# janelia-flyem/flypylib

Hardware: AMD Instinct MI355X
Metric: inference Mvoxels/sec, vgg_like (rf 18, 22^3 coarse -> 88^3 per reference tile), synthetic EM uint8 volume (higher is better)
Workload: dtype f16s; 1 GPU; the 520^3 volume of BASELINE.json's metric (configs[0]'s substack size) per GPU: vgg_like inference, 520x520x520 synthetic uint8 volume, reference tile lattice 102^3 (pitch 88), u8 in / f32 out resident in HBM; tile_in=102, executor=vgg_split_f16, parallelism=z-slab tile sharding x1, no collective, device=AMD Radeon Graphics (gfx950:sramecc+:xnack-)

## Files before the change

flypylib_amd/csrc/vgg_split.hip:

```cpp
#define FPL_F16 1
#include <algorithm>
#include <cmath>

#include "fast_paths.h"
#include "mfma_util.h"
#include "pack_weights.h"
#include <type_traits>
#include "vgg_split_lds.h"
#include "vgg_tiles.h"

namespace {

constexpr int CH = 48;
constexpr int CHP = 24, NPASS = CH / CHP;
constexpr int LO_OFF = CHP * 2;
constexpr int PASS_BYTES = 2 * LO_OFF;
constexpr int VOX = NPASS * PASS_BYTES;
constexpr int KS = (27 * CHP + 31) / 32;
constexpr int KTAB = (KS + 4) / 4 * 4;
constexpr int KTAB_BYTES = 4 * KTAB * 4;
static_assert(CHP % 8 == 0, "a lane's 8 k-slots stay inside one tap");

__host__ __device__ constexpr int64_t chan_off(int ch, int64_t plane) { return (ch / CHP) * plane + (ch % CHP) * 2; }

__device__ __forceinline__ h16x8 pack_relu_split_x(const f32x4 &blk) {
  u32x4 v;
  Pair2 p;
  p = split_pk_relu(blk[0], blk[1]); v[0] = p.hi; v[2] = p.lo;
  p = split_pk_relu(blk[2], blk[3]); v[1] = p.hi; v[3] = p.lo;
  return __builtin_bit_cast(h16x8, v);
}
__device__ __forceinline__ h16x8 pack_relu_split_x(const f32x4 &blk, unsigned &ovf) {
  const h16x8 r = pack_relu_split_x(blk);
  const u32x4 v = __builtin_bit_cast(u32x4, r);
  ovf_note(ovf, pk_max_i16(v[0], v[1]));
  return r;
}

__device__ __forceinline__ f32x4 chain48(const h16x8 (&w)[4], const Frag2 &h01, h16x8 hx, f32x4 acc) {
  acc = mfma16(w[1], h01.hi, acc);
  acc = mfma16(w[0], h01.lo, acc);
  acc = mfma16(w[2], hx, acc);
  acc = mfma16(w[3], hx, acc);
  return mfma16(w[0], h01.hi, acc);
}

__device__ __forceinline__ void store_split12(unsigned char *vox, int64_t plane, int g, const f32x4 (&v)[3],
                                              unsigned &ovf) {
  unsigned hi[6], lo[6];
#pragma unroll
  for (int b = 0; b < 3; ++b) {
    const Pair2 p0 = split_pk(v[b][0], v[b][1], ovf), p1 = split_pk(v[b][2], v[b][3], ovf);
    hi[2 * b] = p0.hi; hi[2 * b + 1] = p1.hi;
    lo[2 * b] = p0.lo; lo[2 * b + 1] = p1.lo;
  }
  unsigned char *d = vox + (g >> 1) * plane + 24 * (g & 1);
  *reinterpret_cast<u32x4_a8 *>(d) = u32x4_a8{hi[0], hi[1], hi[2], hi[3]};
  *reinterpret_cast<u32x2 *>(d + 16) = u32x2{hi[4], hi[5]};
  *reinterpret_cast<u32x4_a8 *>(d + LO_OFF) = u32x4_a8{lo[0], lo[1], lo[2], lo[3]};
  *reinterpret_cast<u32x2 *>(d + LO_OFF + 16) = u32x2{lo[4], lo[5]};
}

constexpr int S_PZ = 4, S_PY = 8, S_PX = 32;
constexpr int S_TZ = 2 * S_PZ + 2, S_TY = 2 * S_PY + 2, S_TX = 2 * S_PX + 2;
constexpr int S_TP = 80;
constexpr int S_TILE = S_TZ * S_TY * S_TP;
constexpr int S_WAVES = 8;
constexpr int S_ROWS = S_TZ * S_TY;
constexpr int S_WROWS = (S_ROWS + S_WAVES - 1) / S_WAVES;
constexpr int S_TASKS = S_PZ * S_PY * 2 / S_WAVES;
constexpr int S_RPT = 3;
static_assert(S_RPT * S_TASKS >= S_WROWS && S_WROWS <= 64, "stem fill schedule");
constexpr int S_SHTAB = 64 * 48;
constexpr int S_SH2 = 4 * 12;
constexpr int S_SMEM = 4 * S_TILE * 2 + 256 * 4 + S_SHTAB * 4 + 2 * S_SH2 * 4;

struct StemSArgs {
  const void *src;
  int64_t SZ, SY, SX;
  int64_t z_hi;
  float mean, sd;
  float c0;
  const float *shtab;
  int64_t p1z0;
  const h16x8 *w1, *w2;
  const float *shift1, *shift2;
  x8::Tensor p1;
  int nbx, nby, nbz;
  int trim;
  unsigned *flag;
  float xlim;
// ... 507 lines not shown
constexpr int WQ = 2;

template <typename Fill, typename SubOff>
__device__ __forceinline__ void conv3s_kloop_f(Fill fill, unsigned char *tile,
                                               const unsigned *kofftab, const unsigned char *wglobal,
                                               unsigned vbase, SubOff sub_off, f32x4 (&acc)[4][3],
                                               int tid) {
  const int lane = tid & 63, wave = tid >> 6, g = lane >> 4;
  const unsigned *ktab = kofftab + g * KTAB;
#pragma unroll 1
  for (int pass = 0; pass < NPASS; ++pass) {
    if (pass) __syncthreads();
    fill(pass);
    const unsigned char *wl = wglobal + (size_t)pass * KS * 6 * 1024 + lane * 16;
    h16x8 wq[WQ][6];
#pragma unroll
    for (int d = 0; d < WQ; ++d)
#pragma unroll
      for (int f = 0; f < 6; ++f)
        wq[d][f] = *reinterpret_cast<const h16x8 *>(wl + (size_t)(d * 6 + f) * 1024);
    __syncthreads();
    u32x4 kv = *reinterpret_cast<const u32x4 *>(ktab);
    Frag2 bcur[4], bnxt[4];
#pragma unroll
    for (int sub = 0; sub < 4; ++sub) {
      const unsigned char *p = tile + vbase + kv[0] + sub_off(sub);
      bcur[sub].hi = *reinterpret_cast<const h16x8 *>(p);
      bcur[sub].lo = *reinterpret_cast<const h16x8 *>(p + LO_OFF);
    }
#pragma unroll
    for (int s = 0; s < KS; ++s) {
      if ((s + 1) % 4 == 0) kv = *reinterpret_cast<const u32x4 *>(ktab + s + 1);
      const unsigned koff = kv[(s + 1) % 4];
#pragma unroll
      for (int sub = 0; sub < 4; ++sub) {
        const unsigned char *p = tile + vbase + koff + sub_off(sub);
        bnxt[sub].hi = *reinterpret_cast<const h16x8 *>(p);
        bnxt[sub].lo = *reinterpret_cast<const h16x8 *>(p + LO_OFF);
      }
      __builtin_amdgcn_s_setprio(1);
#pragma unroll
      for (int sub = 0; sub < 4; ++sub)
#pragma unroll
        for (int b = 0; b < 3; ++b) acc[sub][b] = mfma16(wq[s % WQ][3 + b], bcur[sub].hi, acc[sub][b]);
#pragma unroll
      for (int sub = 0; sub < 4; ++sub)
#pragma unroll
        for (int b = 0; b < 3; ++b) acc[sub][b] = mfma16(wq[s % WQ][b], bcur[sub].lo, acc[sub][b]);
#pragma unroll
      for (int sub = 0; sub < 4; ++sub)
#pragma unroll
        for (int b = 0; b < 3; ++b) acc[sub][b] = mfma16(wq[s % WQ][b], bcur[sub].hi, acc[sub][b]);
      __builtin_amdgcn_s_setprio(0);
      if (s + WQ < KS) {
#pragma unroll
        for (int f = 0; f < 6; ++f)
          wq[s % WQ][f] = *reinterpret_cast<const h16x8 *>(wl + (size_t)((s + WQ) * 6 + f) * 1024);
      }
#pragma unroll
      for (int sub = 0; sub < 4; ++sub) bcur[sub] = bnxt[sub];
    }
  }
}

template <int TZ, int TY, int TX, typename SubOff>
__device__ __forceinline__ void conv3s_kloop(const unsigned char *act, int AZ, int AY, int AX,
                                             int z0, int y0, int x0, unsigned char *tile,
                                             const unsigned *kofftab, const unsigned char *wglobal,
                                             unsigned vbase, SubOff sub_off, f32x4 (&acc)[4][3],
                                             int tid) {
  const int lane = tid & 63, wave = tid >> 6;
  auto fill = [&](int pass) {
    stage_tile<TZ, TY, TX, PASS_BYTES, PASS_BYTES>(act + (int64_t)pass * AZ * AY * AX * PASS_BYTES, AZ, AY, AX,
                                                   z0, y0, x0, tile, wave, lane);
  };
  conv3s_kloop_f(fill, tile, kofftab, wglobal, vbase, sub_off, acc, tid);
}

constexpr int M_TZ = 6, M_TY = 6, M_TX = 18;
constexpr int M_TILE_BYTES = ((M_TZ * M_TY * M_TX * PASS_BYTES + 1023) / 1024) * 1024;
constexpr int M_SMEM = M_TILE_BYTES + KTAB_BYTES;
static_assert(2 * M_SMEM <= 160 * 1024, "two workgroups must fit one CU");

struct MidXArgs {
  x8::Tensor p1;
  const unsigned char *w3;
  const h16x8 *w4;
  const float *shift3, *shift4;
  x8::Tensor p2;
  x8::Walk walk;
  unsigned *flag;
};

__global__ __launch_bounds__(64 * x8::WAVES, 2) void vggs_mid_pool(MidXArgs a) {
  unsigned *ktab = reinterpret_cast<unsigned *>(smem + 2 * x8::BUF);
  const int tid = threadIdx.x, lane = tid & 63;
  const int wave = __builtin_amdgcn_readfirstlane(tid >> 6);
  const int c = lane & 15, g = lane >> 4;
  x8::ktab_init(ktab, tid);
  const x8::TileDma td = x8::tile_dma_init(wave, lane, a.p1.Y, a.p1.XP, (unsigned)a.p1.part_bytes());
  const int S = (int)gridDim.x >> 3, nbricks = a.walk.bricks();
  const int group = (int)blockIdx.x & 7, slot = (int)blockIdx.x >> 3;
  x8::Cursor cur;
  if (!x8::cursor_first(a.walk, nbricks, group, slot, S, cur)) return;
  const int64_t part = a.p1.part_bytes();
  auto origin = [&](const x8::Cursor &q) {
    return a.p1.p + a.p1.vox(8 * q.bz, 4 * q.by, 16 * q.bx) * 16;
  };
  const int pzl = wave >> 1, pyl = wave & 1;
  const unsigned vb = (unsigned)(((2 * pzl) * x8::ZS + (2 * pyl) * x8::TX + c) * 16);
  auto sub_off = [](int sub) -> unsigned { return (unsigned)((((sub >> 1) & 1) * x8::ZS + (sub & 1) * x8::TX) * 16); };
  unsigned ovf_all = 0u;
  x8::prime(smem, td, origin(cur), part, a.w3, wave, lane);
  for (;;) {
    x8::Cursor nxt = cur;
    const bool has_next = x8::cursor_next(a.walk, slot, S, nxt);
    int zero = 0;
    asm volatile("" : "+s"(zero));
    f32x4 acc[4][3];
#pragma unroll
    for (int b = 0; b < 3; ++b) {
      const f32x4 sh = *reinterpret_cast<const f32x4 *>(a.shift3 + zero + 16 * b + 4 * g);
#pragma unroll
      for (int sub = 0; sub < 4; ++sub) acc[sub][b] = sh;
    }
    x8::conv_block(smem, ktab + 8 * g, td, origin(cur), origin(has_next ? nxt : cur), part, a.w3, vb,
                   sub_off, wave, lane, acc);
    asm volatile("" : "+s"(zero));
    const h16x8 *w4p = a.w4 + zero;
    f32x4 sh4[3];
#pragma unroll
    for (int b = 0; b < 3; ++b)
#pragma unroll
      for (int r = 0; r < 4; ++r) sh4[b][r] = a.shift4[zero + x8::out_channel(b, g, r)];
    h16x8 w4[3][4];
#pragma unroll
    for (int s = 0; s < 4; ++s)
#pragma unroll
      for (int b = 0; b < 3; ++b) w4[b][s] = w4p[(s * 3 + b) * 64 + lane];
    f32x4 pooled[3] = {{0.f, 0.f, 0.f, 0.f}, {0.f, 0.f, 0.f, 0.f}, {0.f, 0.f, 0.f, 0.f}};
    unsigned ovf = 0u;
#pragma unroll
    for (int sub = 0; sub < 4; ++sub) {
      const Frag2 h0 = pack_relu_split(acc[sub][0], acc[sub][1], ovf);
      const h16x8 hx = pack_relu_split_x(acc[sub][2], ovf);
#pragma unroll
      for (int b = 0; b < 3; ++b) {
        const f32x4 a4 = chain48(w4[b], h0, hx, sh4[b]);
#pragma unroll
        for (int r = 0; r < 4; ++r) pooled[b][r] = __builtin_fmaxf(pooled[b][r], a4[r]);
      }
    }
#pragma unroll
    for (int b = 0; b < 3; ++b)
#pragma unroll
      for (int r = 0; r < 4; ++r)
        pooled[b][r] = __builtin_fmaxf(pooled[b][r], __shfl_xor(pooled[b][r], 1));
    const int pz = 4 * cur.bz + pzl, py = 2 * cur.by + pyl, px = 8 * cur.bx + (c >> 1);
    const bool inside = pz < a.p2.Z && py < a.p2.Y && px < a.p2.X;
    if ((c & 1) == 0 && inside)
      x8::store12(a.p2, a.p2.vox(pz, py, px), g, pooled, ovf);
    ovf_all = pk_max_i16(ovf_all, inside ? ovf : 0u);
    if (!has_next) break;
    cur = nxt;
  }
  ovf_commit(ovf_all, a.flag, FPL_RANGE_MID);
}

constexpr int T_W7 = 3 * 6, T_W8 = 3;
__device__ __forceinline__ void head_chain(const f32x4 (&acc)[4][3], const unsigned char *w6p,
                                           const unsigned char *w7p, const unsigned char *w8p, const float *sh6p,
                                           const float *sh7p, float bias8, int lane, unsigned &ovf, float (&logit)[4]) {
  const int c = lane & 15, g = lane >> 4;
  auto frag = [&](const unsigned char *w, int part_, int nfrag, int f) {
    return *reinterpret_cast<const h16x8 *>(w + ((size_t)(part_ * nfrag + f) * 64 + lane) * 16);
  };
#pragma unroll
  for (int sp = 0; sp < 2; ++sp) {
    Frag2 h5[2];
    h16x8 h5x[2];
#pragma unroll
    for (int q = 0; q < 2; ++q) {
      h5[q] = pack_relu_split(acc[2 * sp + q][0], acc[2 * sp + q][1], ovf);
      h5x[q] = pack_relu_split_x(acc[2 * sp + q][2], ovf);
    }
    Frag2 h6[2][3];
#pragma unroll
    for (int s = 0; s < 3; ++s) {
      f32x4 a6[2][2];
#pragma unroll
      for (int bb = 0; bb < 2; ++bb) {
        const int b = 2 * s + bb;
        f32x4 sh;
#pragma unroll
        for (int r = 0; r < 4; ++r) sh[r] = sh6p[16 * b + 4 * g + r];
        h16x8 w6[4];
#pragma unroll
        for (int t = 0; t < 4; ++t) w6[t] = frag(w6p, 0, 0, t * 6 + b);
#pragma unroll
        for (int q = 0; q < 2; ++q) a6[q][bb] = chain48(w6, h5[q], h5x[q], sh);
      }
#pragma unroll
      for (int q = 0; q < 2; ++q) h6[q][s] = pack_relu_split(a6[q][0], a6[q][1], ovf);
    }
    f32x4 a8[2] = {{0.f, 0.f, 0.f, 0.f}, {0.f, 0.f, 0.f, 0.f}};
#pragma unroll
    for (int s = 0; s < 3; ++s) {
      f32x4 a7[2][2];
#pragma unroll
      for (int bb = 0; bb < 2; ++bb) {
        const int b = 2 * s + bb;
        f32x4 sh;
#pragma unroll
        for (int r = 0; r < 4; ++r) sh[r] = sh7p[16 * b + 4 * g + r];
#pragma unroll
        for (int q = 0; q < 2; ++q) a7[q][bb] = sh;
#pragma unroll
        for (int t = 0; t < 3; ++t) {
          const h16x8 wh = frag(w7p, 0, T_W7, t * 6 + b), wl = frag(w7p, 1, T_W7, t * 6 + b);
#pragma unroll
          for (int q = 0; q < 2; ++q) a7[q][bb] = mfma3(wh, wl, h6[q][t], a7[q][bb]);
        }
      }
      const h16x8 w8h = frag(w8p, 0, T_W8, s), w8l = frag(w8p, 1, T_W8, s);
#pragma unroll
      for (int q = 0; q < 2; ++q) a8[q] = mfma3(w8h, w8l, pack_relu_split(a7[q][0], a7[q][1], ovf), a8[q]);
    }
#pragma unroll
    for (int q = 0; q < 2; ++q) logit[2 * sp + q] = __shfl(a8[q][0], c) + bias8;
    __builtin_amdgcn_sched_barrier(0);
  }
}

struct TailSArgs {
  const unsigned char *p2;
  int P2Z, P2Y, P2X;
  const unsigned char *w5;
  const float *shift5;
  int CZ, CY, CX;
  const unsigned char *w6, *w7, *w8;
  const float *shift6, *shift7;
  float bias8;
// ... 28 lines not shown
  }
  auto sub_off = [](int sub) -> unsigned { return (unsigned)(sub * M_TX * PASS_BYTES); };
  conv3s_kloop<M_TZ, M_TY, M_TX>(a.p2, a.P2Z, a.P2Y, a.P2X, cz0, cy0, cx0, tile, kofftab, a.w5,
                                 vbase, sub_off, acc, tid);

  float logit[4];
  unsigned ovf = 0u;
  head_chain(acc, a.w6, a.w7, a.w8, a.shift6, a.shift7, a.bias8, lane, ovf, logit);
  ovf_commit(ovf, a.flag, FPL_RANGE_TAIL);

  const int cz = cz0 + wave, cx = cx0 + c;
#pragma unroll
  for (int sub = 0; sub < 4; ++sub) {
    const int cy = cy0 + sub;
    const float p = 1.f / (1.f + expf(-logit[sub]));
    if (cz < a.CZ && cy < a.CY && cx < a.CX) {
      const int64_t fz0 = 4 * (a.gz0 + cz), fy = 4 * (int64_t)cy + g, fx0 = 4 * (int64_t)cx;
      if (fy < a.VY && fx0 < a.VX) {
        const int nx = (int)(a.VX - fx0 < 4 ? a.VX - fx0 : 4);
#pragma unroll
        for (int dz = 0; dz < 4; ++dz) {
          const int64_t fz = fz0 + dz;
          if (fz >= a.VZ) break;
          float *o = a.dst + ((fz + a.off) * a.DY + fy + a.off) * a.DX + fx0 + a.off;
          if (nx == 4) {
            *reinterpret_cast<f32x4_a4 *>(o) = f32x4_a4{p, p, p, p};
          } else {
            for (int i = 0; i < nx; ++i) o[i] = p;
          }
        }
      }
    }
  }
}

struct TailXArgs {
  x8::Tensor p2;
  const unsigned char *w5;
  const float *shift5;
  int CZ, CY, CX;
  const unsigned char *w6, *w7, *w8;
  const float *shift6, *shift7;
  float bias8;
  float *dst;
  int64_t DY, DX;
  int64_t gz0;
  int64_t VZ, VY, VX;
  int off;
  x8::Walk walk;
  unsigned *flag;
};

__global__ __launch_bounds__(64 * x8::WAVES, 2) void vggs_c5_tail(TailXArgs a) {
  unsigned *ktab = reinterpret_cast<unsigned *>(smem + 2 * x8::BUF);
  const int tid = threadIdx.x, lane = tid & 63;
  const int wave = __builtin_amdgcn_readfirstlane(tid >> 6);
  const int c = lane & 15, g = lane >> 4;
  x8::ktab_init(ktab, tid);
  const x8::TileDma td = x8::tile_dma_init(wave, lane, a.p2.Y, a.p2.XP, (unsigned)a.p2.part_bytes());
  const int S = (int)gridDim.x >> 3, nbricks = a.walk.bricks();
  const int group = (int)blockIdx.x & 7, slot = (int)blockIdx.x >> 3;
  x8::Cursor cur;
  if (!x8::cursor_first(a.walk, nbricks, group, slot, S, cur)) return;
  const int64_t part = a.p2.part_bytes();
  auto origin = [&](const x8::Cursor &q) {
    return a.p2.p + a.p2.vox(8 * q.bz, 4 * q.by, 16 * q.bx) * 16;
  };
  const unsigned vb = (unsigned)((wave * x8::ZS + c) * 16);
  auto sub_off = [](int sub) -> unsigned { return (unsigned)(sub * x8::TX * 16); };
  unsigned ovf_all = 0u;
  x8::prime(smem, td, origin(cur), part, a.w5, wave, lane);
  for (;;) {
    x8::Cursor nxt = cur;
    const bool has_next = x8::cursor_next(a.walk, slot, S, nxt);
    int zero = 0;
    asm volatile("" : "+s"(zero));
    f32x4 acc[4][3];
#pragma unroll
    for (int b = 0; b < 3; ++b) {
      const f32x4 sh = *reinterpret_cast<const f32x4 *>(a.shift5 + zero + 16 * b + 4 * g);
#pragma unroll
      for (int sub = 0; sub < 4; ++sub) acc[sub][b] = sh;
    }
    x8::conv_block(smem, ktab + 8 * g, td, origin(cur), origin(has_next ? nxt : cur), part, a.w5, vb,
                   sub_off, wave, lane, acc);

    unsigned ovf = 0u;
    float logit[4];
    asm volatile("" : "+s"(zero));
    head_chain(acc, a.w6 + zero, a.w7 + zero, a.w8 + zero, a.shift6 + zero, a.shift7 + zero, a.bias8, lane, ovf,
               logit);

    const int cz = 8 * cur.bz + wave, cx = 16 * cur.bx + c;
#pragma unroll
    for (int sub = 0; sub < 4; ++sub) {
      const int cy = 4 * cur.by + sub;
      const float p = 1.f / (1.f + expf(-logit[sub]));
      if (cz < a.CZ && cy < a.CY && cx < a.CX) {
        const int64_t fz0 = 4 * (a.gz0 + cz), fy = 4 * (int64_t)cy + g, fx0 = 4 * (int64_t)cx;
        if (fy < a.VY && fx0 < a.VX) {
          const int nx = (int)(a.VX - fx0 < 4 ? a.VX - fx0 : 4);
#pragma unroll
          for (int dz = 0; dz < 4; ++dz) {
            const int64_t fz = fz0 + dz;
            if (fz >= a.VZ) break;
            float *o = a.dst + ((fz + a.off) * a.DY + fy + a.off) * a.DX + fx0 + a.off;
            if (nx == 4) {
              *reinterpret_cast<f32x4_a4 *>(o) = f32x4_a4{p, p, p, p};
            } else {
              for (int i = 0; i < nx; ++i) o[i] = p;
            }
          }
        }
      }
    }
    ovf_all = pk_max_i16(ovf_all, ovf);
    if (!has_next) break;
    cur = nxt;
  }
  ovf_commit(ovf_all, a.flag, FPL_RANGE_TAIL);
}

constexpr int V2_RZ = M_TZ + 2, V2_RY = M_TY + 2, V2_RX = M_TX + 2;
constexpr int V2_NRAW = V2_RZ * V2_RY * V2_RX;
static_assert(V2_NRAW % 256 == 0, "raw tile pieces per thread");
constexpr int V2_SMEM = M_TILE_BYTES + KTAB_BYTES + V2_NRAW * 4 + 256 * 4;
static_assert(2 * V2_SMEM <= 160 * 1024, "two vgg_like2 workgroups must fit one CU");

struct V2SArgs {
  const void *src;
  int64_t SZ, SY, SX;
  float mean, sd;
  int64_t gz0;
  const h16x8 *wstem;
  const float *shstem;
  float c0;
  const float *shtab;
  const unsigned char *in;
  int IZ, IY, IX;
  const unsigned char *w;
  const float *shift;
  unsigned char *out;
  int OZ, OY, OX;
  BlockGrid bg;
  unsigned *flag;
  float xlim;
};

template <bool STEM, bool POOL, typename SRC>
__global__ __launch_bounds__(256, 2) void vggs2_conv3(V2SArgs a) {
  unsigned char *tile = smem;
  unsigned *kofftab = reinterpret_cast<unsigned *>(smem + M_TILE_BYTES);
  unsigned *rawt = reinterpret_cast<unsigned *>(smem + M_TILE_BYTES + KTAB_BYTES);
  unsigned *lut = rawt + V2_NRAW;
  const int tid = threadIdx.x, lane = tid & 63, wave = tid >> 6;
  const int c = lane & 15, g = lane >> 4;
  int xb, yb, zb;
  if (!brick_coords(a.bg, xb, yb, zb)) return;
  const int x0 = xb * 16, y0 = yb * 4, z0 = zb * 4;
  if (tid < 4 * KTAB) kofftab[tid] = kslot_entry<M_TY, M_TX>(tid);
  int toff[8];
  unsigned ovf = 0u, xmax = 0u;
  if (STEM) {
    auto norm_bits = [&](float raw) -> unsigned {
      const float x = (raw - a.mean) / a.sd;
      const unsigned ax = __builtin_bit_cast(unsigned, x) & 0x7FFFFFFFu;
      xmax = ax > xmax ? ax : xmax;
// ... 496 lines not shown
  if (fpl_vgg_variant(prog) == 2)
    return split2_infer(ctx, st, src, src_dtype, mean, sd, dims, origins, out_sz, zb, ze, dst);
  hipStream_t stream = ctx->stream;
  const int64_t SZ = dims[0], SY = dims[1], SX = dims[2];
  const int64_t VZ = SZ - 14, VY = SY - 14, VX = SX - 14;
  if (VZ <= 0 || VY <= 0 || VX <= 0 || zb >= ze) return 0;
  const int64_t fz_lo = (int64_t)origins[0][zb] - 7;
  const int64_t fz_hi = std::min<int64_t>((int64_t)origins[0][ze - 1] - 7 + out_sz[0], VZ);
  const int64_t cz_lo = fz_lo / 4, cz_hi = ceil_div64(fz_hi, 4);
  const int CY = (int)ceil_div64(VY, 4), CX = (int)ceil_div64(VX, 4);
  const int P2Y = CY + 2, P2X = CX + 2, P1Y = 2 * P2Y + 2, P1X = 2 * P2X + 2;
  const int P1XP = x8_pitch(P1X), P2XP = x8_pitch(P2X);
  const int64_t p1_row_bytes = (int64_t)P1Y * P1XP * VOX;
  const char *budget_env = getenv("FPL_VGG_SCRATCH_MB");
  const int64_t budget = budget_env ? (int64_t)atoll(budget_env) << 20 : (int64_t)64 << 30;
  int64_t cz_chunk = std::max<int64_t>(4, (budget / p1_row_bytes - 6) / 2);
  cz_chunk = std::min<int64_t>(cz_chunk, cz_hi - cz_lo);
  cz_chunk = (cz_chunk + 3) / 4 * 4;
  const char *edge_env = getenv("FPL_VGG_EDGE_BLOCKS");
  const int edge_blocks = edge_env ? atoi(edge_env) != 0 : 1;
  FPL_REQUIRE(ctx, (int64_t)S_TZ * SY * SX < ((int64_t)1 << 31),
              "vgg split path: a %lld x %lld plane is too large for the stem's 31-bit row "
              "offsets", (long long)SY, (long long)SX);
  {
    const int64_t max_rows = (((int64_t)1 << 32) / 16 / ((int64_t)P1Y * P1XP) - (x8::TZ + 2));
    FPL_REQUIRE(ctx, max_rows >= 14,
                "vgg split path: a %lld x %lld plane is too large for the tile loader's 32-bit "
                "offsets", (long long)SY, (long long)SX);
    cz_chunk = std::min<int64_t>(cz_chunk, std::max<int64_t>(4, ((max_rows - 6) / 2) / 4 * 4));
  }
  DevTemp tmp(ctx);
  unsigned *flag;
  FPL_TRY(fpl_range_flag(ctx, &flag));
  x8::Tensor p1 = {nullptr, (int)(2 * cz_chunk + 6), P1Y, P1X, P1XP}, p2 = {nullptr, (int)(cz_chunk + 2), P2Y, P2X, P2XP};
  void *p1v, *p2v;
  FPL_TRY(tmp.alloc((size_t)(p1.bytes() + p1.slack_bytes()), &p1v));
  FPL_TRY(tmp.alloc((size_t)(p2.bytes() + p2.slack_bytes()), &p2v));
  void *dumpv;
  FPL_TRY(tmp.alloc(256, &dumpv));
  const unsigned pgrid = (unsigned)std::max(8, ctx->n_cu / 8 * 8);
  const unsigned char *F = st->frags;
  const float *S = st->shifts;
  for (int64_t c0 = cz_lo; c0 < cz_hi; c0 += cz_chunk) {
    const int CZ = (int)std::min<int64_t>(cz_chunk, cz_hi - c0);
    const int P2Z = CZ + 2, P1Z = 2 * P2Z + 2;
    p1 = x8::Tensor{(unsigned char *)p1v, P1Z, P1Y, P1X, P1XP};
    p2 = x8::Tensor{(unsigned char *)p2v, P2Z, P2Y, P2X, P2XP};
    FPL_HIP(ctx, hipMemsetAsync(p1.p + p1.bytes(), 0, (size_t)p1.slack_bytes(), stream));
    FPL_HIP(ctx, hipMemsetAsync(p2.p + p2.bytes(), 0, (size_t)p2.slack_bytes(), stream));
    {
      StemSArgs a;
      a.src = src; a.SZ = SZ; a.SY = SY; a.SX = SX; a.mean = mean; a.sd = sd;
      a.p1z0 = 2 * c0;
      a.z_hi = std::min<int64_t>(SZ, 4 * (c0 + CZ) + 14);
      a.w1 = (const h16x8 *)(F + st->off_w[0]);
      a.w2 = (const h16x8 *)(F + st->off_w[1]);
      a.shift1 = S + st->off_s[0]; a.shift2 = S + st->off_s[1];
      a.c0 = 0.f; a.shtab = nullptr;
      if (src_dtype == FPL_U8) {
        a.w1 = (const h16x8 *)st->w1_int; a.shtab = st->shift1_int;
        a.c0 = st->int_c0;
      }
      a.p1 = p1;
      a.flag = flag; a.xlim = st->xlim; a.dump = (unsigned char *)dumpv;
      a.nbx = (int)ceil_div64(P1X, S_PX); a.nby = (int)ceil_div64(P1Y, S_PY);
      a.nbz = (int)ceil_div64(P1Z, S_PZ);
      a.trim = edge_blocks;
      const unsigned grid = (unsigned)std::min<int64_t>((int64_t)a.nbx * a.nby * a.nbz,
                                                        (int64_t)ctx->n_cu);
      TimedLaunch tl(ctx, "vggs_stem_pool");
      if (src_dtype == FPL_U8)
        vggs_stem_pool<uint8_t><<<grid, 64 * S_WAVES, S_SMEM, stream>>>(a);
      else
        vggs_stem_pool<float><<<grid, 64 * S_WAVES, S_SMEM, stream>>>(a);
    }
    {
      MidXArgs a;
      a.p1 = p1;
      a.w3 = F + st->off_w[2];
      a.w4 = (const h16x8 *)(F + st->off_w[3]);
      a.shift3 = S + st->off_s[2]; a.shift4 = S + st->off_s[3];
      a.p2 = p2;
      a.flag = flag;
      a.walk = x8::Walk{(int)ceil_div64(P2X, 8), (int)ceil_div64(P2Y, 2), (int)ceil_div64(P2Z, 4)};
      TimedLaunch tl(ctx, "vggs_mid_pool");
      vggs_mid_pool<<<pgrid, 64 * x8::WAVES, x8::SMEM, stream>>>(a);
    }
    {
      TailXArgs a;
      a.p2 = p2;
      a.w5 = F + st->off_w[4]; a.shift5 = S + st->off_s[4];
      a.CZ = CZ; a.CY = CY; a.CX = CX;
      a.w6 = F + st->off_w[5]; a.w7 = F + st->off_w[6]; a.w8 = F + st->off_w[7];
      a.shift6 = S + st->off_s[5]; a.shift7 = S + st->off_s[6]; a.bias8 = st->bias8;
      a.dst = dst; a.DY = SY; a.DX = SX; a.gz0 = c0;
      a.VZ = std::min<int64_t>(fz_hi, VZ); a.VY = VY; a.VX = VX; a.off = 7;
      a.flag = flag;
      a.walk = x8::Walk{(int)ceil_div64(CX, 16), (int)ceil_div64(CY, 4), (int)ceil_div64(CZ, 8)};
      TimedLaunch tl(ctx, "vggs_c5_tail");
      vggs_c5_tail<<<pgrid, 64 * x8::WAVES, x8::SMEM, stream>>>(a);
    }
    FPL_HIP(ctx, hipGetLastError());
  }
  return 0;
}
```

flypylib_amd/csrc/vgg_split_lds.h:

```cpp
#pragma once
#include "mfma_util.h"
#include "vgg_tiles.h"

namespace x8 {

constexpr int CQ = 8, NQ = 6;
constexpr int KQ = 7;
constexpr int BZ = 8, BY = 4, BX = 16;
constexpr int TZ = BZ + 2, TY = BY + 2, TX = BX + 2;
constexpr int ZS = 118;
constexpr int PLANE = (TZ - 1) * ZS + TY * TX;
constexpr int CHUNKS = (2 * PLANE + 63) / 64;
constexpr int TILE_BYTES = CHUNKS * 1024;
constexpr int WFRAGS = KQ * 6;
constexpr int WBYTES = WFRAGS * 1024;
constexpr int BUF = TILE_BYTES + WBYTES;
constexpr int KTAB_BYTES = 4 * 8 * 4;
constexpr int SMEM = 2 * BUF + KTAB_BYTES;
constexpr int WAVES = 8;
constexpr int TCH = (CHUNKS + WAVES - 1) / WAVES;
constexpr int WCH = (WFRAGS + WAVES - 1) / WAVES;
static_assert((ZS - 2 * TX - 2) % 16 == 0 && (TX - 2) % 16 == 0, "conflict-free tap offsets");
static_assert(SMEM <= 160 * 1024, "one workgroup per CU");
static_assert(PLANE % 2 == 0, "");

struct Tensor {
  unsigned char *p;
  int Z, Y, X;
  int XP;
  __host__ __device__ int64_t part_bytes() const { return (int64_t)Z * Y * XP * 16; }
  __host__ __device__ int64_t pass_bytes() const { return 2 * part_bytes(); }
  __host__ __device__ int64_t bytes() const { return NQ * pass_bytes(); }
  __host__ __device__ int64_t slack_bytes() const { return ((int64_t)(TZ + 1) * Y * XP + 64) * 16; }
  __host__ __device__ int64_t vox(int z, int y, int x) const { return ((int64_t)z * Y + y) * XP + x; }
};

struct Walk {
  int nbx, nby, nbz;
  __host__ __device__ int bricks() const { return ((nbx + 3) / 4) * ((nby + 3) / 4) * ((nbz + 1) / 2); }
};

struct TileDma {
  unsigned off[TCH];
};
__device__ __forceinline__ TileDma tile_dma_init(int wave, int lane, int SY, int SX, unsigned part_bytes) {
  TileDma d;
#pragma unroll
  for (int i = 0; i < TCH; ++i) {
    int slot = 64 * (wave + WAVES * i) + lane;
    slot = slot < 2 * PLANE ? slot : 2 * PLANE - 1;
    const int part = slot >= PLANE;
    const int s = slot - part * PLANE;
    const int tz = s / ZS;
    int rem = s - tz * ZS;
    rem = rem < TY * TX ? rem : TY * TX - 1;
    const int ty = rem / TX, tx = rem - ty * TX;
    d.off[i] = (unsigned)(((tz * SY + ty) * SX + tx) * 16) + (part ? part_bytes : 0u);
  }
  return d;
}

constexpr int NCH = CHUNKS + WFRAGS;
constexpr int DCH = (NCH + WAVES - 1) / WAVES;
constexpr int HCH = DCH / 2;
static_assert(TCH == 5 && 8 * 4 + 4 < CHUNKS && 8 * 4 + 5 >= CHUNKS, "chunk deal: i = 4 splits at wave 5");
static_assert(DCH % 2 == 0, "two batches");
__device__ __forceinline__ void dma_batch(const TileDma &d, int half, int wave, int lane, const unsigned char *org,
                                          const unsigned char *wpass, unsigned char *buf) {
#pragma unroll
  for (int k = 0; k < HCH; ++k) {
    const int i = HCH * half + k;
    int j = wave + WAVES * i;
    j = j < NCH ? j : NCH - 1;
    const bool tile = i < TCH - 1 || (i < TCH && j < CHUNKS);
    const unsigned char *base = tile ? org : wpass + (j - CHUNKS) * 1024;
    const unsigned off = tile ? d.off[i < TCH ? i : 0] : (unsigned)lane * 16u;
    glds16(base + off, buf + j * 1024);
  }
}

__device__ __forceinline__ void ktab_init(unsigned *ktab, int tid) {
  if (tid < 32) {
    const int g = tid >> 3, s = tid & 7;
    const int tap = 4 * s + g;
    ktab[tid] = tap < 27 ? (unsigned)(((tap / 9) * ZS + ((tap / 3) % 3) * TX + tap % 3) * 16) : 0u;
  }
}

template <typename SubOff, typename Issue>
__device__ __forceinline__ void pass_kloop(const unsigned char *buf, const unsigned *ktab_g, unsigned vb,
                                           SubOff sub_off, Issue issue, int lane, f32x4 (&acc)[4][3]) {
  const unsigned char *wl = buf + TILE_BYTES + lane * 16;
  const u32x4 k0 = *reinterpret_cast<const u32x4 *>(ktab_g), k1 = *reinterpret_cast<const u32x4 *>(ktab_g + 4);
  Frag2 bcur[4], bnxt[4];
  h16x8 wcur[6], wnxt[6];
#pragma unroll
  for (int sub = 0; sub < 4; ++sub) {
    const unsigned char *p = buf + vb + k0[0] + sub_off(sub);
    bcur[sub].hi = *reinterpret_cast<const h16x8 *>(p);
    bcur[sub].lo = *reinterpret_cast<const h16x8 *>(p + PLANE * 16);
  }
#pragma unroll
  for (int f = 0; f < 6; ++f) wcur[f] = *reinterpret_cast<const h16x8 *>(wl + f * 1024);
#pragma unroll
  for (int s = 0; s < KQ; ++s) {
    __builtin_amdgcn_sched_barrier(0);
    __builtin_amdgcn_s_setprio(1);
#pragma unroll
    for (int sub = 0; sub < 4; ++sub)
#pragma unroll
      for (int b = 0; b < 3; ++b) acc[sub][b] = mfma16(wcur[3 + b], bcur[sub].hi, acc[sub][b]);
    __builtin_amdgcn_sched_barrier(0);
    if (s + 1 < KQ) {
      const unsigned koff = s + 1 < 4 ? k0[(s + 1) & 3] : k1[(s + 1) & 3];
#pragma unroll
      for (int sub = 0; sub < 4; ++sub) {
        const unsigned char *p = buf + vb + koff + sub_off(sub);
        bnxt[sub].hi = *reinterpret_cast<const h16x8 *>(p);
        bnxt[sub].lo = *reinterpret_cast<const h16x8 *>(p + PLANE * 16);
      }
    }
    __builtin_amdgcn_sched_barrier(0);
#pragma unroll
    for (int sub = 0; sub < 4; ++sub)
#pragma unroll
      for (int b = 0; b < 3; ++b) acc[sub][b] = mfma16(wcur[b], bcur[sub].lo, acc[sub][b]);
    __builtin_amdgcn_sched_barrier(0);
    if (s + 1 < KQ) {
#pragma unroll
      for (int f = 0; f < 6; ++f) wnxt[f] = *reinterpret_cast<const h16x8 *>(wl + ((s + 1) * 6 + f) * 1024);
    }
    issue(s);
    __builtin_amdgcn_sched_barrier(0);
#pragma unroll
    for (int sub = 0; sub < 4; ++sub)
#pragma unroll
      for (int b = 0; b < 3; ++b) acc[sub][b] = mfma16(wcur[b], bcur[sub].hi, acc[sub][b]);
    __builtin_amdgcn_s_setprio(0);
    __builtin_amdgcn_sched_barrier(0);
    if (s + 1 < KQ) {
#pragma unroll
      for (int sub = 0; sub < 4; ++sub) bcur[sub] = bnxt[sub];
#pragma unroll
      for (int f = 0; f < 6; ++f) wcur[f] = wnxt[f];
    }
  }
}

template <typename SubOff>
__device__ __forceinline__ void conv_block(unsigned char *smem, const unsigned *ktab_g, const TileDma &td,
                                           const unsigned char *org_cur, const unsigned char *org_nxt,
                                           int64_t part_bytes, const unsigned char *wglobal, unsigned vb,
                                           SubOff sub_off, int wave, int lane, f32x4 (&acc)[4][3]) {
#pragma unroll 1
  for (int pp = 0; pp < NQ / 2; ++pp) {
#pragma unroll
    for (int h = 0; h < 2; ++h) {
      const int pass = 2 * pp + h;
      unsigned char *buf = smem + h * BUF, *other = smem + (h ^ 1) * BUF;
      const bool more = pass + 1 < NQ;
      const unsigned char *torg = more ? org_cur + (int64_t)(pass + 1) * 2 * part_bytes : org_nxt;
      const unsigned char *tw = wglobal + (size_t)(more ? pass + 1 : 0) * WBYTES;
      auto issue = [&](int s) {
        if (s == 0 || s == 3) {
          __builtin_amdgcn_s_setprio(0);
          dma_batch(td, s == 3, wave, lane, torg, tw, other);
          __builtin_amdgcn_s_setprio(1);
        }
      };
      pass_kloop(buf, ktab_g, vb, sub_off, issue, lane, acc);
      __syncthreads();
    }
  }
}

__device__ __forceinline__ void prime(unsigned char *smem, const TileDma &td, const unsigned char *org,
                                      int64_t part_bytes, const unsigned char *wglobal, int wave, int lane) {
#pragma unroll
  for (int half = 0; half < 2; ++half) dma_batch(td, half, wave, lane, org, wglobal, smem);
  __syncthreads();
}

__device__ __forceinline__ void walk_decode(const Walk &w, int i, int &bx, int &by, int &bz) {
  const int layer = w.nbx * w.nby * 2;
  const int kz = i / layer;
  int r = i - kz * layer;
  const int wz = min(2, w.nbz - 2 * kz);
  const int rowb = w.nbx * 4 * wz;
  const int ky = r / rowb;
  r -= ky * rowb;
  const int wy = min(4, w.nby - 4 * ky);
  const int bb = 4 * wy * wz;
  const int kx = r / bb;
  r -= kx * bb;
  const int wx = min(4, w.nbx - 4 * kx);
  bx = 4 * kx + r % wx;
  r /= wx;
  by = 4 * ky + r % wy;
  bz = 2 * kz + r / wy;
}
struct Cursor {
  int i, iend;
  int bx, by, bz;
};
__device__ __forceinline__ bool cursor_first(const Walk &w, int , int group, int slot, int S, Cursor &c) {
  const int total = w.nbx * w.nby * w.nbz, per = (total + 7) / 8;
  c.i = group * per + slot;
  c.iend = (group + 1) * per < total ? (group + 1) * per : total;
  if (c.i >= c.iend) return false;
  walk_decode(w, c.i, c.bx, c.by, c.bz);
  return true;
}
__device__ __forceinline__ bool cursor_next(const Walk &w, int , int S, Cursor &c) {
  c.i += S;
  if (c.i >= c.iend) return false;
  walk_decode(w, c.i, c.bx, c.by, c.bz);
  return true;
}

__host__ __device__ constexpr int out_channel(int b, int g, int r) { return b < 2 ? 8 * g + 4 * b + r : 32 + 4 * g + r; }
__device__ __forceinline__ void store12(const Tensor &t, int64_t vox, int g, const f32x4 (&v)[3], unsigned &ovf) {
  unsigned hi[6], lo[6];
#pragma unroll
  for (int b = 0; b < 3; ++b) {
    const Pair2 p0 = split_pk(v[b][0], v[b][1], ovf), p1 = split_pk(v[b][2], v[b][3], ovf);
    hi[2 * b] = p0.hi; hi[2 * b + 1] = p1.hi;
    lo[2 * b] = p0.lo; lo[2 * b + 1] = p1.lo;
  }
  const int64_t part = t.part_bytes();
  unsigned char *q = t.p + (int64_t)g * 2 * part + vox * 16;
  unsigned char *h = t.p + (int64_t)(4 + (g >> 1)) * 2 * part + vox * 16 + 8 * (g & 1);
  *reinterpret_cast<u32x4 *>(q) = u32x4{hi[0], hi[1], hi[2], hi[3]};
  *reinterpret_cast<u32x4 *>(q + part) = u32x4{lo[0], lo[1], lo[2], lo[3]};
  *reinterpret_cast<u32x2 *>(h) = u32x2{hi[4], hi[5]};
  *reinterpret_cast<u32x2 *>(h + part) = u32x2{lo[4], lo[5]};
}

__device__ __forceinline__ void store12_sel(const Tensor &t, int64_t vox, int g, const f32x4 (&v)[3],
                                            unsigned &ovf, bool valid, unsigned char *dump) {
  unsigned hi[6], lo[6], o2 = 0u;
#pragma unroll
  for (int b = 0; b < 3; ++b) {
    const Pair2 p0 = split_pk(v[b][0], v[b][1], o2), p1 = split_pk(v[b][2], v[b][3], o2);
    hi[2 * b] = p0.hi; hi[2 * b + 1] = p1.hi;
    lo[2 * b] = p0.lo; lo[2 * b + 1] = p1.lo;
  }
  ovf_note(ovf, valid ? o2 : 0u);
  const int64_t part = t.part_bytes();
  unsigned char *q = t.p + (int64_t)g * 2 * part + vox * 16;
  unsigned char *h = t.p + (int64_t)(4 + (g >> 1)) * 2 * part + vox * 16 + 8 * (g & 1);
  *reinterpret_cast<u32x4 *>(valid ? q : dump) = u32x4{hi[0], hi[1], hi[2], hi[3]};
  *reinterpret_cast<u32x4 *>(valid ? q + part : dump + 16) = u32x4{lo[0], lo[1], lo[2], lo[3]};
  *reinterpret_cast<u32x2 *>(valid ? h : dump + 32) = u32x2{hi[4], hi[5]};
  *reinterpret_cast<u32x2 *>(valid ? h + part : dump + 48) = u32x2{lo[4], lo[5]};
}

}
```

Baseline: 15570 Mvoxels/s.

## Cover mid-layer ragged edges with narrow and z-thin tile geometries

Adds two alternative LDS tile geometries (x-narrow and z-thin) to the mid conv+pool kernel, which are used when a full brick would mostly compute padding past the volume edge. The last partial x-column of bricks and a one-plane z remainder are re-tiled into differently shaped bricks, so fewer wasted MFMAs run on out-of-range voxels. To support this, the work is split into full and edge lists per group, the DMA offsets are switched per brick kind, and the LDS part stride is fixed at PL. The cost is extra branching, more register pressure for three TileDma sets, and a more complex cursor decode.

```diff
diff --git a/flypylib_amd/csrc/vgg_mid_cover.h b/flypylib_amd/csrc/vgg_mid_cover.h
--- /dev/null
+++ b/flypylib_amd/csrc/vgg_mid_cover.h
@@ -0,0 +1,56 @@
+#pragma once
+#include "vgg_split_lds.h"
+
+struct MidCover {
+  x8::Walk walk;
+  int nx_cols, nx_rows, nx_lay;
+  int th_rows;
+  __host__ __device__ int full() const { return walk.nbx * walk.nby * walk.nbz; }
+  __host__ __device__ int narrow() const { return nx_cols * nx_rows * nx_lay; }
+  __host__ __device__ int edge() const { return narrow() + walk.nbx * th_rows; }
+};
+
+struct MidCursor {
+  int l, n;
+  int nf, e0;
+  int kind, bx, by, bz;
+};
+__host__ __device__ inline void mid_decode(const MidCover &m, int f0, MidCursor &c) {
+  if (c.l < c.nf) {
+    c.kind = 0;
+    x8::walk_decode(m.walk, f0 + c.l, c.bx, c.by, c.bz);
+    return;
+  }
+  int e = c.e0 + c.l - c.nf;
+  if (e < m.narrow()) {
+    c.kind = 1;
+    c.bx = e % m.nx_cols;
+    e /= m.nx_cols;
+    c.by = e % m.nx_rows;
+    c.bz = e / m.nx_rows;
+  } else {
+    e -= m.narrow();
+    c.kind = 2;
+    c.bx = e % m.walk.nbx;
+    c.by = e / m.walk.nbx;
+    c.bz = m.walk.nbz;
+  }
+}
+
+inline MidCover mid_cover(int P2Z, int P2Y, int P2X, bool edge) {
+  MidCover m{};
+  m.walk = x8::Walk{(P2X + 7) / 8, (P2Y + 1) / 2, (P2Z + 3) / 4};
+  if (!edge) return m;
+  const int rx = P2X % 8;
+  if (rx != 0 && (rx + 1) / 2 * ((P2Y + 7) / 8) < m.walk.nby) {
+    m.nx_cols = (rx + 1) / 2;
+    m.nx_rows = (P2Y + 7) / 8;
+    m.nx_lay = m.walk.nbz;
+    m.walk.nbx -= 1;
+  }
+  if (P2Z % 4 == 1 && (P2Y + 6) / 7 < m.walk.nby) {
+    m.th_rows = (P2Y + 6) / 7;
+    m.walk.nbz -= 1;
+  }
+  return m;
+}
diff --git a/flypylib_amd/csrc/vgg_split.hip b/flypylib_amd/csrc/vgg_split.hip
--- a/flypylib_amd/csrc/vgg_split.hip
+++ b/flypylib_amd/csrc/vgg_split.hip
@@ -7,6 +7,7 @@
 #include "pack_weights.h"
 #include <type_traits>
 #include "vgg_split_lds.h"
+#include "vgg_mid_cover.h"
 #include "vgg_tiles.h"
 
 namespace {
@@ -680,13 +681,17 @@
 constexpr int M_SMEM = M_TILE_BYTES + KTAB_BYTES;
 static_assert(2 * M_SMEM <= 160 * 1024, "two workgroups must fit one CU");
 
+using GeoNarrow = x8::Geo<10, 18, 6, 109>;
+using GeoThin = x8::Geo<4, 16, 18, 294>;
+static_assert((GeoThin::ZS - 2 * GeoThin::TX - 2) % 16 == 0, "z-thin taps conflict-free as the full block's");
+
 struct MidXArgs {
   x8::Tensor p1;
   const unsigned char *w3;
   const h16x8 *w4;
   const float *shift3, *shift4;
   x8::Tensor p2;
-  x8::Walk walk;
+  MidCover cover;
   unsigned *flag;
 };
 
@@ -695,24 +700,49 @@
   const int tid = threadIdx.x, lane = tid & 63;
   const int wave = __builtin_amdgcn_readfirstlane(tid >> 6);
   const int c = lane & 15, g = lane >> 4;
-  x8::ktab_init(ktab, tid);
-  const x8::TileDma td = x8::tile_dma_init(wave, lane, a.p1.Y, a.p1.XP, (unsigned)a.p1.part_bytes());
-  const int S = (int)gridDim.x >> 3, nbricks = a.walk.bricks();
+  if (tid < 96) {
+    const int gs = tid & 31;
+    ktab[tid] = tid < 32 ? x8::ktab_entry<x8::GeoFull>(gs >> 3, gs & 7)
+              : tid < 64 ? x8::ktab_entry<GeoNarrow>(gs >> 3, gs & 7)
+                         : x8::ktab_entry<GeoThin>(gs >> 3, gs & 7);
+  }
+  const MidCover &m = a.cover;
+  const int S = (int)gridDim.x >> 3;
   const int group = (int)blockIdx.x & 7, slot = (int)blockIdx.x >> 3;
-  x8::Cursor cur;
-  if (!x8::cursor_first(a.walk, nbricks, group, slot, S, cur)) return;
+  const int F = m.full(), E = m.edge(), pf = (F + 7) / 8, pe = (E + 7) / 8;
+  const int f0 = group * pf;
+  MidCursor cur;
+  cur.nf = max(0, min(pf, F - f0));
+  cur.e0 = group * pe;
+  cur.n = cur.nf + max(0, min(pe, E - cur.e0));
+  cur.l = slot;
+  if (cur.l >= cur.n) return;
+  mid_decode(m, f0, cur);
   const int64_t part = a.p1.part_bytes();
-  auto origin = [&](const x8::Cursor &q) {
-    return a.p1.p + a.p1.vox(8 * q.bz, 4 * q.by, 16 * q.bx) * 16;
+  auto origin = [&](const MidCursor &q) {
+    const int z = q.kind == 2 ? 8 * m.walk.nbz : 8 * q.bz;
+    const int y = q.kind == 0 ? 4 * q.by : q.kind == 1 ? 16 * q.by : 14 * q.by;
+    const int x = q.kind == 1 ? 16 * m.walk.nbx + 4 * q.bx : 16 * q.bx;
+    return a.p1.p + a.p1.vox(z, y, x) * 16;
+  };
+  auto tile_dma = [&](int kind) {
+    const unsigned pb = (unsigned)a.p1.part_bytes();
+    const x8::TileDma d0 = x8::tile_dma_init<x8::GeoFull>(wave, lane, a.p1.Y, a.p1.XP, pb);
+    const x8::TileDma d1 = x8::tile_dma_init<GeoNarrow>(wave, lane, a.p1.Y, a.p1.XP, pb);
+    const x8::TileDma d2 = x8::tile_dma_init<GeoThin>(wave, lane, a.p1.Y, a.p1.XP, pb);
+    return x8::tile_dma_sel(kind == 0, d0, x8::tile_dma_sel(kind == 1, d1, d2));
   };
   const int pzl = wave >> 1, pyl = wave & 1;
-  const unsigned vb = (unsigned)(((2 * pzl) * x8::ZS + (2 * pyl) * x8::TX + c) * 16);
-  auto sub_off = [](int sub) -> unsigned { return (unsigned)((((sub >> 1) & 1) * x8::ZS + (sub & 1) * x8::TX) * 16); };
   unsigned ovf_all = 0u;
-  x8::prime(smem, td, origin(cur), part, a.w3, wave, lane);
+  const x8::TileDma td0 = x8::tile_dma_init<x8::GeoFull>(wave, lane, a.p1.Y, a.p1.XP, (unsigned)a.p1.part_bytes());
+  x8::prime(smem, tile_dma(cur.kind), origin(cur), part, a.w3, wave, lane);
   for (;;) {
-    x8::Cursor nxt = cur;
-    const bool has_next = x8::cursor_next(a.walk, slot, S, nxt);
+    MidCursor nxt = cur;
+    nxt.l += S;
+    const bool has_next = nxt.l < nxt.n;
+    if (has_next) mid_decode(m, f0, nxt);
+    const int kind_nxt = has_next ? nxt.kind : cur.kind;
+    const unsigned char *org_nxt = has_next ? origin(nxt) : origin(cur);
     int zero = 0;
     asm volatile("" : "+s"(zero));
     f32x4 acc[4][3];
@@ -722,8 +752,33 @@
 #pragma unroll
       for (int sub = 0; sub < 4; ++sub) acc[sub][b] = sh;
     }
-    x8::conv_block(smem, ktab + 8 * g, td, origin(cur), origin(has_next ? nxt : cur), part, a.w3, vb,
-                   sub_off, wave, lane, acc);
+    if (cur.kind == 0) {
+      using G = x8::GeoFull;
+      const unsigned vb = (unsigned)(((2 * pzl) * G::ZS + (2 * pyl) * G::TX + c) * 16);
+      auto sub_off = [](int sub) -> unsigned { return (unsigned)((((sub >> 1) & 1) * G::ZS + (sub & 1) * G::TX) * 16); };
+      if (kind_nxt == 0) {
+        x8::conv_block<false>(smem, ktab + 8 * g, td0, td0, origin(cur), org_nxt, part, a.w3, vb, sub_off, wave, lane,
+                              acc);
+      } else {
+        const x8::TileDma tdn = tile_dma(kind_nxt);
+        x8::conv_block<true>(smem, ktab + 8 * g, td0, tdn, origin(cur), org_nxt, part, a.w3, vb, sub_off, wave, lane,
+                             acc);
+      }
+    } else if (cur.kind == 1) {
+      using G = GeoNarrow;
+      const unsigned vb = (unsigned)(((2 * pzl) * G::ZS + c * G::TX + 2 * pyl) * 16);
+      auto sub_off = [](int sub) -> unsigned { return (unsigned)((((sub >> 1) & 1) * G::ZS + (sub & 1)) * 16); };
+      const x8::TileDma td = tile_dma(1), tdn = tile_dma(kind_nxt);
+      x8::conv_block<true>(smem, ktab + 32 + 8 * g, td, tdn, origin(cur), org_nxt, part, a.w3, vb, sub_off, wave, lane,
+                           acc);
+    } else {
+      using G = GeoThin;
+      const unsigned vb = (unsigned)((2 * min(wave, 6) * G::TX + c) * 16);
+      auto sub_off = [](int sub) -> unsigned { return (unsigned)((((sub >> 1) & 1) * G::ZS + (sub & 1) * G::TX) * 16); };
+      const x8::TileDma td = tile_dma(2), tdn = tile_dma(kind_nxt);
+      x8::conv_block<true>(smem, ktab + 64 + 8 * g, td, tdn, origin(cur), org_nxt, part, a.w3, vb, sub_off, wave, lane,
+                           acc);
+    }
     asm volatile("" : "+s"(zero));
     const h16x8 *w4p = a.w4 + zero;
     f32x4 sh4[3];
@@ -754,8 +809,17 @@
 #pragma unroll
       for (int r = 0; r < 4; ++r)
         pooled[b][r] = __builtin_fmaxf(pooled[b][r], __shfl_xor(pooled[b][r], 1));
-    const int pz = 4 * cur.bz + pzl, py = 2 * cur.by + pyl, px = 8 * cur.bx + (c >> 1);
-    const bool inside = pz < a.p2.Z && py < a.p2.Y && px < a.p2.X;
+    int pz = 4 * cur.bz + pzl, py = 2 * cur.by + pyl, px = 8 * cur.bx + (c >> 1);
+    bool live = true;
+    if (cur.kind == 1) {
+      py = 8 * cur.by + (c >> 1);
+      px = 8 * m.walk.nbx + 2 * cur.bx + pyl;
+    } else if (cur.kind == 2) {
+      pz = 4 * m.walk.nbz;
+      py = 7 * cur.by + wave;
+      live = wave < 7;
+    }
+    const bool inside = live && pz < a.p2.Z && py < a.p2.Y && px < a.p2.X;
     if ((c & 1) == 0 && inside)
       x8::store12(a.p2, a.p2.vox(pz, py, px), g, pooled, ovf);
     ovf_all = pk_max_i16(ovf_all, inside ? ovf : 0u);
@@ -950,7 +1014,7 @@
 #pragma unroll
       for (int sub = 0; sub < 4; ++sub) acc[sub][b] = sh;
     }
-    x8::conv_block(smem, ktab + 8 * g, td, origin(cur), origin(has_next ? nxt : cur), part, a.w5, vb,
+    x8::conv_block<false>(smem, ktab + 8 * g, td, td, origin(cur), origin(has_next ? nxt : cur), part, a.w5, vb,
                    sub_off, wave, lane, acc);
 
     unsigned ovf = 0u;
@@ -1613,7 +1677,7 @@
       a.shift3 = S + st->off_s[2]; a.shift4 = S + st->off_s[3];
       a.p2 = p2;
       a.flag = flag;
-      a.walk = x8::Walk{(int)ceil_div64(P2X, 8), (int)ceil_div64(P2Y, 2), (int)ceil_div64(P2Z, 4)};
+      a.cover = mid_cover(P2Z, P2Y, P2X, edge_blocks);
       TimedLaunch tl(ctx, "vggs_mid_pool");
       vggs_mid_pool<<<pgrid, 64 * x8::WAVES, x8::SMEM, stream>>>(a);
     }
diff --git a/flypylib_amd/csrc/vgg_split_lds.h b/flypylib_amd/csrc/vgg_split_lds.h
--- a/flypylib_amd/csrc/vgg_split_lds.h
+++ b/flypylib_amd/csrc/vgg_split_lds.h
@@ -10,19 +10,29 @@
 constexpr int TZ = BZ + 2, TY = BY + 2, TX = BX + 2;
 constexpr int ZS = 118;
 constexpr int PLANE = (TZ - 1) * ZS + TY * TX;
-constexpr int CHUNKS = (2 * PLANE + 63) / 64;
+constexpr int PL = 1184;
+constexpr int CHUNKS = 2 * PL / 64;
 constexpr int TILE_BYTES = CHUNKS * 1024;
 constexpr int WFRAGS = KQ * 6;
 constexpr int WBYTES = WFRAGS * 1024;
 constexpr int BUF = TILE_BYTES + WBYTES;
-constexpr int KTAB_BYTES = 4 * 8 * 4;
+constexpr int NGEO = 3;
+constexpr int KTAB_BYTES = NGEO * 4 * 8 * 4;
 constexpr int SMEM = 2 * BUF + KTAB_BYTES;
 constexpr int WAVES = 8;
 constexpr int TCH = (CHUNKS + WAVES - 1) / WAVES;
 constexpr int WCH = (WFRAGS + WAVES - 1) / WAVES;
 static_assert((ZS - 2 * TX - 2) % 16 == 0 && (TX - 2) % 16 == 0, "conflict-free tap offsets");
 static_assert(SMEM <= 160 * 1024, "one workgroup per CU");
-static_assert(PLANE % 2 == 0, "");
+static_assert(PLANE <= PL && 2 * PL % 64 == 0, "");
+
+template <int TZ_, int TY_, int TX_, int ZS_>
+struct Geo {
+  static constexpr int TZ = TZ_, TY = TY_, TX = TX_, ZS = ZS_;
+  static constexpr int PLANE = (TZ - 1) * ZS + TY * TX;
+  static_assert(ZS >= TY * TX && PLANE <= PL, "tile plane fits the LDS part");
+};
+using GeoFull = Geo<TZ, TY, TX, ZS>;
 
 struct Tensor {
   unsigned char *p;
@@ -43,19 +53,31 @@
 struct TileDma {
   unsigned off[TCH];
 };
+template <class G = GeoFull>
 __device__ __forceinline__ TileDma tile_dma_init(int wave, int lane, int SY, int SX, unsigned part_bytes) {
   TileDma d;
 #pragma unroll
   for (int i = 0; i < TCH; ++i) {
-    int slot = 64 * (wave + WAVES * i) + lane;
-    slot = slot < 2 * PLANE ? slot : 2 * PLANE - 1;
-    const int part = slot >= PLANE;
-    const int s = slot - part * PLANE;
-    const int tz = s / ZS;
-    int rem = s - tz * ZS;
-    rem = rem < TY * TX ? rem : TY * TX - 1;
-    const int ty = rem / TX, tx = rem - ty * TX;
+    const int slot = 64 * (wave + WAVES * i) + lane;
+    const int part = slot >= PL;
+    int s = slot - part * PL;
+    s = s < G::PLANE ? s : G::PLANE - 1;
+    const int tz = s / G::ZS;
+    int rem = s - tz * G::ZS;
+    rem = rem < G::TY * G::TX ? rem : G::TY * G::TX - 1;
+    const int ty = rem / G::TX, tx = rem - ty * G::TX;
     d.off[i] = (unsigned)(((tz * SY + ty) * SX + tx) * 16) + (part ? part_bytes : 0u);
+  }
+  return d;
+}
+
+__device__ __forceinline__ TileDma tile_dma_sel(bool p, const TileDma &a, const TileDma &b) {
+  TileDma d;
+#pragma unroll
+  for (int i = 0; i < TCH; ++i) {
+    unsigned x = a.off[i], y = b.off[i];
+    asm volatile("" : "+v"(x), "+v"(y));
+    d.off[i] = p ? x : y;
   }
   return d;
 }
@@ -79,12 +101,13 @@
   }
 }
 
+template <class G>
+__device__ __forceinline__ unsigned ktab_entry(int g, int s) {
+  const int tap = 4 * s + g;
+  return tap < 27 ? (unsigned)(((tap / 9) * G::ZS + ((tap / 3) % 3) * G::TX + tap % 3) * 16) : 0u;
+}
 __device__ __forceinline__ void ktab_init(unsigned *ktab, int tid) {
-  if (tid < 32) {
-    const int g = tid >> 3, s = tid & 7;
-    const int tap = 4 * s + g;
-    ktab[tid] = tap < 27 ? (unsigned)(((tap / 9) * ZS + ((tap / 3) % 3) * TX + tap % 3) * 16) : 0u;
-  }
+  if (tid < 32) ktab[tid] = ktab_entry<GeoFull>(tid >> 3, tid & 7);
 }
 
 template <typename SubOff, typename Issue>
@@ -98,7 +121,7 @@
   for (int sub = 0; sub < 4; ++sub) {
     const unsigned char *p = buf + vb + k0[0] + sub_off(sub);
     bcur[sub].hi = *reinterpret_cast<const h16x8 *>(p);
-    bcur[sub].lo = *reinterpret_cast<const h16x8 *>(p + PLANE * 16);
+    bcur[sub].lo = *reinterpret_cast<const h16x8 *>(p + PL * 16);
   }
 #pragma unroll
   for (int f = 0; f < 6; ++f) wcur[f] = *reinterpret_cast<const h16x8 *>(wl + f * 1024);
@@ -117,7 +140,7 @@
       for (int sub = 0; sub < 4; ++sub) {
         const unsigned char *p = buf + vb + koff + sub_off(sub);
         bnxt[sub].hi = *reinterpret_cast<const h16x8 *>(p);
-        bnxt[sub].lo = *reinterpret_cast<const h16x8 *>(p + PLANE * 16);
+        bnxt[sub].lo = *reinterpret_cast<const h16x8 *>(p + PL * 16);
       }
     }
     __builtin_amdgcn_sched_barrier(0);
@@ -147,9 +170,9 @@
   }
 }
 
-template <typename SubOff>
+template <bool TWO, typename SubOff>
 __device__ __forceinline__ void conv_block(unsigned char *smem, const unsigned *ktab_g, const TileDma &td,
-                                           const unsigned char *org_cur, const unsigned char *org_nxt,
+                                           const TileDma &td_nxt, const unsigned char *org_cur, const unsigned char *org_nxt,
                                            int64_t part_bytes, const unsigned char *wglobal, unsigned vb,
                                            SubOff sub_off, int wave, int lane, f32x4 (&acc)[4][3]) {
 #pragma unroll 1
@@ -164,7 +187,10 @@
       auto issue = [&](int s) {
         if (s == 0 || s == 3) {
           __builtin_amdgcn_s_setprio(0);
-          dma_batch(td, s == 3, wave, lane, torg, tw, other);
+          if constexpr (TWO)
+            dma_batch(tile_dma_sel(more, td, td_nxt), s == 3, wave, lane, torg, tw, other);
+          else
+            dma_batch(td, s == 3, wave, lane, torg, tw, other);
           __builtin_amdgcn_s_setprio(1);
         }
       };
@@ -181,7 +207,7 @@
   __syncthreads();
 }
 
-__device__ __forceinline__ void walk_decode(const Walk &w, int i, int &bx, int &by, int &bz) {
+__host__ __device__ inline void walk_decode(const Walk &w, int i, int &bx, int &by, int &bz) {
   const int layer = w.nbx * w.nby * 2;
   const int kz = i / layer;
   int r = i - kz * layer;
```

Result: faster. 16150 Mvoxels/s, median of 6 (+3.7%).
